# DataZooDE/anofox-forecast

Measured on AMD Instinct MI355X. Metric: series/sec fit+forecast, AutoETS h=28 on M5-shape batches, higher is better.
Workload: dtype f64

## Files before the change

### anofox-forecast_amd/csrc/ets_device.hpp

```cpp
#pragma once
#include <hip/hip_runtime.h>
#include <type_traits>
#include "det_math.hpp"
#include "nm.hpp"

namespace anofox {

enum { C_NONE = 0, C_ADD = 1, C_MUL = 2 };

constexpr double ETS_TOL = 1.0e-10;
constexpr double ETS_HUGEN = 1.0e10;
constexpr double ETS_LN2 = 0.693147180559945309417232121458;
constexpr double PAR_LO = 1.0e-4, PAR_HI = 0.9999, PHI_LO = 0.8, PHI_HI = 0.98;
constexpr int ETS_MERGED_LDS_PERIOD = 16;
constexpr int ETS_LDS_PERIOD = 64;
constexpr int ETS_MAX_PERIOD = 2048;

struct SeriesView {
    const double *y;
    size_t ld;
    int len;
    int wave_len;
    int wave_min_len;
    int rows;
    const double *yb;
    int col;
};

__device__ __forceinline__ int wave_max_i32(int v)
{
#pragma unroll
    for (int o = 32; o >= 1; o >>= 1) { int w = __shfl_xor(v, o); v = w > v ? w : v; }
    return v;
}
__device__ __forceinline__ int wave_min_i32(int v)
{
#pragma unroll
    for (int o = 32; o >= 1; o >>= 1) { int w = __shfl_xor(v, o); v = w < v ? w : v; }
    return v;
}

enum { YT_F64 = 0, YT_F32 = 1, YT_U16 = 2 };
template <class YT> struct YtCode;
template <> struct YtCode<double> { static constexpr int value = YT_F64; };
template <> struct YtCode<float> { static constexpr int value = YT_F32; };
template <> struct YtCode<unsigned short> { static constexpr int value = YT_U16; };
#ifndef ANOFOX_DM_RETRY
#define ANOFOX_DM_RETRY 0
#endif
#ifndef ANOFOX_TWO_BLOCK
#define ANOFOX_TWO_BLOCK 1
#endif
#ifndef ANOFOX_S_DM
#define ANOFOX_S_DM 8
#endif
#ifndef ANOFOX_S_GEN
#define ANOFOX_S_GEN 16
#endif
#ifndef ANOFOX_S_HBM_RING_COMPACT
#define ANOFOX_S_HBM_RING_COMPACT 16
#endif
#ifndef ANOFOX_S_COMPACT_MUL
#define ANOFOX_S_COMPACT_MUL 2
#endif
#ifndef ANOFOX_S_COMPACT_MUL_ADD
#define ANOFOX_S_COMPACT_MUL_ADD 1
#endif
#ifndef ANOFOX_K4_S_SEAS
#define ANOFOX_K4_S_SEAS 8
#endif
template <int ERR, int TREND, bool DAMPED, int SEAS>
struct EtsCfg {
    static constexpr int E = ERR, T = TREND, S = SEAS;
    static constexpr bool D = DAMPED;
    static constexpr int DIM = 1 + (TREND != C_NONE) + (SEAS != C_NONE) + (DAMPED ? 1 : 0);
    static constexpr bool ADDITIVE = (ERR == C_ADD) && (TREND != C_MUL) && (SEAS != C_MUL);
    static constexpr bool CLASSIC = false;
};

struct EtsPar { double alpha, bstar, phi, beta, gamma; DmPowLane pl; DmPowNear1 pc; };
struct EtsState { double l, b, sse, mant; int eacc; int bad; double f; double dlo, dhi, bmin; double rfar; };

template <class Cfg>
__device__ __forceinline__ void ets_unpack(const double (&x)[Cfg::DIM], EtsPar &p)
{
    int k = 0;
    p.alpha = x[k++];
    p.bstar = 0.0;
    double gstar = 0.0;
    p.phi = 1.0;
    if constexpr (Cfg::T != C_NONE) p.bstar = x[k++];
    if constexpr (Cfg::S != C_NONE) gstar = x[k++];
    if constexpr (Cfg::D) p.phi = x[k++];
    p.beta = p.alpha * p.bstar;
    p.gamma = gstar * (1.0 - p.alpha);
}

template <class Cfg, bool NEAR = false>
__device__ __forceinline__ void ets_step(const EtsPar &p, EtsState &st, double y, double &s)
{
    if constexpr (Cfg::ADDITIVE) {
        double phib = 0.0, q = st.l;
        if constexpr (Cfg::T == C_ADD) {
            phib = Cfg::D ? p.phi * st.b : st.b;
            q = st.l + phib;
        }
        double f = q;
        if constexpr (Cfg::S == C_ADD) f = q + s;
        double e = y - f;
        st.sse = fma(e, e, st.sse);
        st.l = fma(p.alpha, e, q);
        st.f = f;
        if constexpr (Cfg::T == C_ADD) st.b = fma(p.beta, e, phib);
        if constexpr (Cfg::S == C_ADD) s = fma(p.gamma, e, s);
    } else {
        double phib = 0.0, q = st.l;
        if constexpr (Cfg::T == C_ADD) {
            phib = Cfg::D ? p.phi * st.b : st.b;
            q = st.l + phib;
        } else if constexpr (Cfg::T == C_MUL) {
            if constexpr (Cfg::D) {
                const double r = st.b - 1.0;
                phib = dm_pow_near1(r, p.pc);
                if constexpr (NEAR) st.rfar = __builtin_fmax(st.rfar, fabs(r));
                else if (!(fabs(r) <= DM_POW_NEAR1_R)) {
                    if (!(st.b >= 0x1p-1000 && st.b <= 0x1p+1000)) st.bad = 1;
                    phib = dm_pow_step(st.b, p.phi, p.pl);
                }
            } else {
                st.bmin = __builtin_fmin(st.bmin, st.b);
                phib = st.b;
            }
            q = st.l * phib;
        }
        double f = q;
        if constexpr (Cfg::S == C_ADD) f = q + s;
        else if constexpr (Cfg::S == C_MUL) f = q * s;
        st.f = f;
        auto recip = [&](const double d) __attribute__((always_inline)) {
            const double ad = fabs(d);
            st.dlo = __builtin_fmin(st.dlo, ad);
            st.dhi = __builtin_fmax(st.dhi, ad);
            return dm_recip(d);
        };
        if constexpr (Cfg::E == C_MUL) {
            static_assert(Cfg::S != C_ADD, "multiplicative error with an additive season is not a valid spec");
            const double rf = recip(f);
            const double eps = (y - f) * rf;
            st.mant = st.mant * fabs(f);
            st.sse = fma(eps, eps, st.sse);
            const double qe = q * eps;
            st.l = fma(p.alpha, qe, q);
            if constexpr (Cfg::T == C_ADD) st.b = fma(p.beta, qe, phib);
            else if constexpr (Cfg::T == C_MUL) st.b = fma(p.beta, phib * eps, phib);
            if constexpr (Cfg::S == C_MUL) s = fma(p.gamma, s * eps, s);
        } else {
            const double e = y - f;
            st.sse = fma(e, e, st.sse);
            if constexpr (Cfg::S == C_MUL && Cfg::T == C_MUL) {
                const double R = recip(f * st.l);
                const double esl = e * (R * q);
                const double es = esl * st.l;
                const double sl = s * st.l;
                st.l = fma(p.alpha, es, q);
                st.b = fma(p.beta, esl, phib);
                s = fma(p.gamma, e * (R * sl), s);
            } else if constexpr (Cfg::S == C_MUL) {
                const double R = recip(f);
                const double es = e * (R * q);
                st.l = fma(p.alpha, es, q);
                if constexpr (Cfg::T == C_ADD) st.b = fma(p.beta, es, phib);
                s = fma(p.gamma, e * (R * s), s);
            } else {
                static_assert(Cfg::T == C_MUL, "general class: a multiplicative component");
                const double rl = recip(st.l);
                st.l = fma(p.alpha, e, q);
                st.b = fma(p.beta, e * rl, phib);
                if constexpr (Cfg::S == C_ADD) s = fma(p.gamma, e, s);
            }
        }
    }
}

template <class Cfg>
__device__ __forceinline__ void ets_renorm(EtsState &st)
{
    if constexpr (Cfg::E == C_MUL) {
        int ex;
        st.mant = frexp(st.mant, &ex);
        st.eacc += ex;
    }
}

template <class Cfg>
__device__ __forceinline__ double ets_objective_value(const EtsState &st, int n)
{
    if (st.bad || !(fabs(st.sse) <= 1.7976931348623157e308)) return __builtin_huge_val();
    if constexpr (!Cfg::ADDITIVE) {
        constexpr double D_LO = Cfg::E == C_MUL ? 0x1p-120 : 0x1p-1000, D_HI = Cfg::E == C_MUL ? 0x1p+120 : 0x1p+1000;
        if (n > 0 && !(st.dlo >= D_LO && st.dhi <= D_HI)) return __builtin_huge_val();
        if constexpr (Cfg::T == C_MUL && !Cfg::D) { if (n > 0 && !(st.bmin > 0.0)) return __builtin_huge_val(); }
    }
    double lik = (double)n * dm_log(st.sse);
    if constexpr (Cfg::E == C_MUL) lik = lik + 2.0 * (dm_log(st.mant) + (double)st.eacc * ETS_LN2);
    if (lik != lik) return __builtin_huge_val();
    if (lik < -1.0e10) lik = -1.0e10;
    return lik;
}

struct EtsInit {
    double l0, b0;
    const double *fig;
    size_t fig_ld;
    int m;
};

struct EtsFinalOut {
    double *yhat; int h; double *sse_out;
    double *fitted; size_t fitted_ld; double *states; size_t states_ld;
    double mean; double *var_out;
};

template <class Cfg, int MS, int K, bool FINAL, class YT = double>
__device__ __forceinline__ void ets_pass(const SeriesView &v, const EtsInit &in,
                                         const double (&cand)[K][Cfg::DIM], double (&fout)[K],
                                         double *ring, const EtsFinalOut *fin)
{
    static_assert((Cfg::S == C_NONE) == (MS == 0), "MS == 0 iff no seasonal component");
    const int lane = threadIdx.x & (NM_BLOCK - 1);
    EtsPar par[K];
    EtsState st[K];
#pragma unroll
    for (int k = 0; k < K; k++) {
        ets_unpack<Cfg>(cand[k], par[k]);
        if constexpr (Cfg::T == C_MUL && Cfg::D) { par[k].pl = dm_pow_lane(); dm_pow_near1_coef(par[k].phi, par[k].pc); }
        st[k].l = in.l0; st[k].b = in.b0; st[k].sse = 0.0; st[k].mant = 1.0; st[k].eacc = 0; st[k].bad = 0;
        st[k].f = 0.0; st[k].dlo = __builtin_huge_val(); st[k].dhi = 0.0; st[k].bmin = __builtin_huge_val(); st[k].rfar = 0.0;

    }
    const double *yp = v.yb;
    const unsigned col_bytes = (unsigned)v.col * (unsigned)sizeof(YT);
    const size_t ld = v.ld;

    const int wave_len = __builtin_amdgcn_readfirstlane(v.wave_len);
    const int wave_min_len = __builtin_amdgcn_readfirstlane(v.wave_min_len);
    const int row_max = __builtin_amdgcn_readfirstlane(v.rows) - 1;
    constexpr int S_WIDE = std::is_same_v<YT, double> ? 1 : (Cfg::ADDITIVE ? ANOFOX_S_COMPACT_MUL_ADD : ANOFOX_S_COMPACT_MUL);
    constexpr int S_FULL = (Cfg::ADDITIVE ? (K == 4 ? (MS > 0 ? ANOFOX_K4_S_SEAS : 16) : 32) : ((Cfg::T == C_MUL && Cfg::D) ? ANOFOX_S_DM : ANOFOX_S_GEN)) * S_WIDE;
    constexpr int S_HBM_CAP = (MS == -2 && !FINAL && !std::is_same_v<YT, double>) ? ANOFOX_S_HBM_RING_COMPACT : 8;
    constexpr int S_TARGET = ((MS == -2 || MS == -4) && K == 1 && S_FULL > S_HBM_CAP) ? S_HBM_CAP : S_FULL;
    constexpr int S = (MS > 0) ? ((S_TARGET / MS > 0 ? S_TARGET / MS : 1) * MS) : S_TARGET;
    typedef std::conditional_t<std::is_same_v<YT, unsigned short>, unsigned, YT> ybuf_t;
    auto widen = [](const ybuf_t x) __attribute__((always_inline)) { return (double)x; };
    ybuf_t cur[S], nxt[S];
    typedef unsigned int u32x2_t __attribute__((ext_vector_type(2)));
    const size_t row_bytes = ld * sizeof(YT);
    const size_t total_bytes = (size_t)(row_max + 1) * row_bytes;
    const int rows_total = row_max + 1;
    auto load_block = [&](ybuf_t (&buf)[S], const int row0) __attribute__((always_inline)) {
        unsigned nrec;
        size_t off;
        if constexpr (Cfg::ADDITIVE) {
            const unsigned rows_left = row0 < rows_total ? (unsigned)(rows_total - row0) : 0u;
            const unsigned long long rem = (unsigned long long)rows_left * (unsigned long long)(unsigned)row_bytes;
            nrec = (unsigned)(rem >> 32) != 0u ? 0xffffffffu : (unsigned)rem;
            off = rows_left ? (size_t)((unsigned long long)(unsigned)row0 * (unsigned long long)(unsigned)row_bytes) : (size_t)0;
        } else {
            const size_t o = (size_t)row0 * row_bytes;
            const size_t rem = o < total_bytes ? total_bytes - o : 0;
            nrec = rem > 0xffffffffull ? 0xffffffffu : (unsigned)rem;
            off = rem ? o : 0;
        }
        const auto rsrc = __builtin_amdgcn_make_buffer_rsrc((void *)((const char *)yp + off), 0, nrec, 0x00020000);
#pragma unroll
        for (int j = 0; j < S; j++) {
            if constexpr (std::is_same_v<YT, double>) {
                const u32x2_t w = __builtin_amdgcn_raw_buffer_load_b64(rsrc, col_bytes, (unsigned)(j * row_bytes), 0);
                buf[j] = __builtin_bit_cast(double, w);
            } else if constexpr (std::is_same_v<YT, float>) {
                const unsigned w = __builtin_amdgcn_raw_buffer_load_b32(rsrc, col_bytes, (unsigned)(j * row_bytes), 0);
                buf[j] = __builtin_bit_cast(float, w);
            } else {
                buf[j] = (unsigned)__builtin_amdgcn_raw_buffer_load_b16(rsrc, col_bytes, (unsigned)(j * row_bytes), 0);
            }
        }
    };
    load_block(cur, 0);
    double var_acc = 0.0;
    auto keep_fit = [&](const int t, const double yv) __attribute__((always_inline)) {
        if constexpr (FINAL) {
            if (fin->fitted && t < v.len) fin->fitted[(size_t)t * fin->fitted_ld] = st[0].f;
            const double dv = yv - fin->mean;
            var_acc += dv * dv;
        }
    };

    if constexpr (MS >= 0) {
        constexpr int MR = MS > 0 ? MS : 1;
        double s[K][MR];
        if constexpr (MS > 0) {
#pragma unroll
            for (int j = 0; j < MS; j++) {
                double f0 = in.fig[(size_t)j * in.fig_ld];
#pragma unroll
                for (int k = 0; k < K; k++) s[k][j] = f0;
            }
        } else {
#pragma unroll
            for (int k = 0; k < K; k++) s[k][0] = 0.0;
        }
        auto run_block = [&](const ybuf_t (&buf)[S], const int base, auto pred_tag) __attribute__((always_inline)) {
            constexpr bool PRED = decltype(pred_tag)::value;
            if constexpr (ANOFOX_DM_RETRY && Cfg::T == C_MUL && Cfg::D && K == 1 && !PRED && !FINAL) {
                const EtsState st0 = st[0];
                double s0[MR];
#pragma unroll
                for (int jj = 0; jj < MR; jj++) s0[jj] = s[0][jj];
                st[0].rfar = 0.0;
#pragma unroll
                for (int j = 0; j < S; j++) {
                    ets_step<Cfg, true>(par[0], st[0], widen(buf[j]), s[0][MS > 0 ? j % MR : 0]);
                    if ((j & 3) == 3 || j == S - 1) ets_renorm<Cfg>(st[0]);
                }
                const bool again = v.len > 0 && (!(st[0].rfar <= DM_POW_NEAR1_R) || st[0].b != st[0].b);
                if (__builtin_amdgcn_ballot_w64(again) == 0ull) return;
                st[0] = st0;
#pragma unroll
                for (int jj = 0; jj < MR; jj++) s[0][jj] = s0[jj];
            }
#pragma unroll
            for (int j = 0; j < S; j++) {
                if (!PRED || base + j < v.len) {
#pragma unroll
                    for (int k = 0; k < K; k++) {
                        ets_step<Cfg>(par[k], st[k], widen(buf[j]), s[k][MS > 0 ? j % MR : 0]);
                        if ((j & 3) == 3 || j == S - 1) ets_renorm<Cfg>(st[k]);
                    }
                    keep_fit(base + j, widen(buf[j]));
                }
            }
        };
        int base = 0;
        constexpr bool TWO = ANOFOX_TWO_BLOCK == 2 || (ANOFOX_TWO_BLOCK == 1 && Cfg::ADDITIVE);
        if constexpr (TWO) {
            for (; base + 2 * S <= wave_min_len; base += 2 * S) {
                load_block(nxt, base + S);
                run_block(cur, base, std::false_type{});
                load_block(cur, base + 2 * S);
                run_block(nxt, base + S, std::false_type{});
            }
        }
        for (; base < wave_len; base += S) {
            load_block(nxt, base + S);
            if (base + S <= wave_min_len) run_block(cur, base, std::false_type{});
            else run_block(cur, base, std::true_type{});
#pragma unroll
            for (int j = 0; j < S; j++) cur[j] = nxt[j];
        }
        if constexpr (FINAL) {
            if constexpr (MS > 0) {
                if (fin->states && v.len > 0) {
#pragma unroll
                    for (int jj = 0; jj < MS; jj++) fin->states[(size_t)(2 + jj) * fin->states_ld] = s[0][jj];
                }
            }
            double pp = par[0].phi, phistar = par[0].phi;
            for (int i = 0; i < fin->h; i++) {
                double f;
                if constexpr (Cfg::T == C_NONE) f = st[0].l;
                else if constexpr (Cfg::T == C_ADD) f = st[0].l + phistar * st[0].b;
                else f = (st[0].b > 0.0) ? st[0].l * dm_pow_pos(st[0].b, phistar) : __builtin_nan("");
                if constexpr (MS > 0) {
                    const int j = (v.len + i) % MS;
                    double sv = s[0][0];
#pragma unroll
                    for (int jj = 1; jj < MS; jj++) sv = (j == jj) ? s[0][jj] : sv;
                    f = (Cfg::S == C_ADD) ? f + sv : f * sv;
                }
                if (v.len > 0) fin->yhat[i] = f;
                pp = pp * par[0].phi;
                phistar = phistar + pp;
            }
        }
    } else {
        constexpr bool LANE_M = MS <= -3;
        static_assert(!LANE_M || K == 1, "per-lane periods: one candidate per lane");
        const int m = LANE_M ? in.m : __builtin_amdgcn_readfirstlane(in.m);
        const int m_max = LANE_M ? __builtin_amdgcn_readfirstlane(wave_max_i32(in.m)) : m;
        for (int j = 0; j < m_max; j++) {
            if (LANE_M && j >= m) continue;
            double f0 = in.fig[(size_t)j * in.fig_ld];
#pragma unroll
            for (int k = 0; k < K; k++) ring[(k * m + j) * NM_BLOCK + lane] = f0;
        }
        int j = 0;
        constexpr bool HBM_RING = (MS == -2 || MS == -4);
        if constexpr (HBM_RING && K == 1) {
            static_assert(2 * S <= ((MS == -2 && !FINAL) ? ETS_LDS_PERIOD : ETS_MERGED_LDS_PERIOD), "the ring prefetch needs periods of at least two blocks");
            double rc[S], rn[S];
            auto ring_load = [&](double (&buf)[S], int j0) __attribute__((always_inline)) {
#pragma unroll
                for (int i = 0; i < S; i++) {
                    buf[i] = ring[(size_t)j0 * NM_BLOCK + lane];
                    j0 = (j0 + 1 == m) ? 0 : j0 + 1;
                }
                return j0;
            };
            int jn = ring_load(rc, 0);
            int base = 0;
            for (; base < wave_len; base += S) {
                load_block(nxt, base + S);
                const int jnn = ring_load(rn, jn);
                const bool full = base + S <= wave_min_len;
#pragma unroll
                for (int i = 0; i < S; i++) {
                    if (full || base + i < v.len) {
                        double sv = rc[i];
                        ets_step<Cfg>(par[0], st[0], widen(cur[i]), sv);
                        if ((i & 3) == 3 || i == S - 1) ets_renorm<Cfg>(st[0]);
                        ring[(size_t)j * NM_BLOCK + lane] = sv;
                        keep_fit(base + i, widen(cur[i]));
                    }
                    j = (j + 1 == m) ? 0 : j + 1;
                }
#pragma unroll
                for (int i = 0; i < S; i++) { cur[i] = nxt[i]; rc[i] = rn[i]; }
                jn = jnn;
            }
        } else {
        auto ring_block = [&](const int base, const bool full) __attribute__((always_inline)) {
#pragma unroll
            for (int i = 0; i < S; i++) {
                if (full || base + i < v.len) {
#pragma unroll
                    for (int k = 0; k < K; k++) {
                        double sv = ring[(k * m + j) * NM_BLOCK + lane];
                        ets_step<Cfg>(par[k], st[k], widen(cur[i]), sv);
                        if ((i & 3) == 3 || i == S - 1) ets_renorm<Cfg>(st[k]);
                        ring[(k * m + j) * NM_BLOCK + lane] = sv;
                    }
                    keep_fit(base + i, widen(cur[i]));
                }
                j = (j + 1 == m) ? 0 : j + 1;
            }
        };
        int base = 0;
        for (; base < wave_len; base += S) {
            load_block(nxt, base + S);
            ring_block(base, base + S <= wave_min_len);
#pragma unroll
            for (int i = 0; i < S; i++) cur[i] = nxt[i];
        }
        }
        if constexpr (FINAL) {
            if (fin->states && v.len > 0)
                for (int jj = 0; jj < m; jj++) fin->states[(size_t)(2 + jj) * fin->states_ld] = ring[(0 * m + jj) * NM_BLOCK + lane];
            double pp = par[0].phi, phistar = par[0].phi;
            for (int i = 0; i < fin->h; i++) {
                double f;
                if constexpr (Cfg::T == C_NONE) f = st[0].l;
                else if constexpr (Cfg::T == C_ADD) f = st[0].l + phistar * st[0].b;
                else f = (st[0].b > 0.0) ? st[0].l * dm_pow_pos(st[0].b, phistar) : __builtin_nan("");
                const int jj = (v.len + i) % m;
                double sv = ring[(0 * m + jj) * NM_BLOCK + lane];
                f = (Cfg::S == C_ADD) ? f + sv : f * sv;
                if (v.len > 0) fin->yhat[i] = f;
                pp = pp * par[0].phi;
                phistar = phistar + pp;
            }
        }
    }
#pragma unroll
    for (int k = 0; k < K; k++) {
        ets_renorm<Cfg>(st[k]);
        fout[k] = ets_objective_value<Cfg>(st[k], v.len);
    }
    if constexpr (FINAL) {
        if (fin->sse_out && v.len > 0) *fin->sse_out = st[0].sse;
        if (fin->var_out) *fin->var_out = var_acc;
        if (fin->states && v.len > 0) { fin->states[0] = st[0].l; fin->states[fin->states_ld] = Cfg::T != C_NONE ? st[0].b : __builtin_nan(""); }
    }
}

template <class Cfg, int MS, int CPL, class YT = double>
struct EtsModel {
    static constexpr int DIM = Cfg::DIM;
    SeriesView v;
    EtsInit in;
    double *ring;
    __device__ void bounds(double (&lo)[DIM], double (&hi)[DIM], double (&x0)[DIM]) const
    {
        int k = 0;
        lo[k] = PAR_LO; hi[k] = PAR_HI; x0[k] = 0.3; k++;
        if constexpr (Cfg::T != C_NONE) { lo[k] = PAR_LO; hi[k] = PAR_HI; x0[k] = 0.1; k++; }
        if constexpr (Cfg::S != C_NONE) { lo[k] = PAR_LO; hi[k] = PAR_HI; x0[k] = 0.1; k++; }
        if constexpr (Cfg::D) { lo[k] = PHI_LO; hi[k] = PHI_HI; x0[k] = 0.9; k++; }
    }
    __device__ double eval1(const double (&x)[DIM]) const
    {
        double c1[1][DIM], f1[1];
#pragma unroll
        for (int i = 0; i < DIM; i++) c1[0][i] = x[i];
        ets_pass<Cfg, MS, 1, false, YT>(v, in, c1, f1, ring, nullptr);
        return f1[0];
    }
    __device__ void eval(const double (&cand)[NM_K][DIM], double (&f)[NM_K]) const
    {
        if constexpr (CPL == NM_K) {
            ets_pass<Cfg, MS, NM_K, false, YT>(v, in, cand, f, ring, nullptr);
        } else {
            const int sub = threadIdx.x & 3;
            double mine[1][DIM], f1[1];
#pragma unroll
            for (int i = 0; i < DIM; i++)
                mine[0][i] = sub == 0 ? cand[0][i] : (sub == 1 ? cand[1][i] : (sub == 2 ? cand[2][i] : cand[3][i]));
            ets_pass<Cfg, MS, 1, false, YT>(v, in, mine, f1, ring, nullptr);
            const int base = (threadIdx.x & (NM_BLOCK - 1)) & ~3;
#pragma unroll
            for (int k = 0; k < NM_K; k++) f[k] = __shfl(f1[0], base + k);
        }
    }
};

}
```

Baseline: 79800.

## Add optional per-row refill ring for y loads and halve renorm frequency

Adds an ANOFOX_ROW_RING option that replaces the double-buffered cur/nxt block prefetch with a single buffer, where each slot is refilled with the next block's row right after it is consumed. The goal is to cut register pressure from holding two blocks. Separately, the state renormalisation in every ETS step loop now runs every 8 steps instead of every 4, which applies unconditionally. The ring path defaults to off, so only the renorm change is active by default; it reduces work but leaves mantissa accumulation unrenormalised over longer stretches.

```diff
diff --git a/anofox-forecast_amd/csrc/ets_device.hpp b/anofox-forecast_amd/csrc/ets_device.hpp
--- a/anofox-forecast_amd/csrc/ets_device.hpp
+++ b/anofox-forecast_amd/csrc/ets_device.hpp
@@ -50,6 +50,9 @@
 #endif
 #ifndef ANOFOX_TWO_BLOCK
 #define ANOFOX_TWO_BLOCK 1
+#endif
+#ifndef ANOFOX_ROW_RING
+#define ANOFOX_ROW_RING 0
 #endif
 #ifndef ANOFOX_S_DM
 #define ANOFOX_S_DM 8
@@ -251,13 +254,16 @@
     constexpr int S_TARGET = ((MS == -2 || MS == -4) && K == 1 && S_FULL > S_HBM_CAP) ? S_HBM_CAP : S_FULL;
     constexpr int S = (MS > 0) ? ((S_TARGET / MS > 0 ? S_TARGET / MS : 1) * MS) : S_TARGET;
     typedef std::conditional_t<std::is_same_v<YT, unsigned short>, unsigned, YT> ybuf_t;
-    auto widen = [](const ybuf_t x) __attribute__((always_inline)) { return (double)x; };
-    ybuf_t cur[S], nxt[S];
+    constexpr bool ROW_RING = ANOFOX_ROW_RING && K == 1 && !ANOFOX_DM_RETRY && !(ANOFOX_ROW_RING == 2 && Cfg::T == C_MUL && Cfg::D);
+    constexpr bool RAW_RING = ROW_RING && ((MS >= 0 && Cfg::T == C_MUL && Cfg::D) || MS == -1 || MS == -3);
+    typedef std::conditional_t<RAW_RING, YT, ybuf_t> yslot_t;
+    auto widen = [](const yslot_t x) __attribute__((always_inline)) { return (double)x; };
+    yslot_t cur[S], nxt[S];
     typedef unsigned int u32x2_t __attribute__((ext_vector_type(2)));
     const size_t row_bytes = ld * sizeof(YT);
     const size_t total_bytes = (size_t)(row_max + 1) * row_bytes;
     const int rows_total = row_max + 1;
-    auto load_block = [&](ybuf_t (&buf)[S], const int row0) __attribute__((always_inline)) {
+    auto block_rsrc = [&](const int row0) __attribute__((always_inline)) {
         unsigned nrec;
         size_t off;
         if constexpr (Cfg::ADDITIVE) {
@@ -271,21 +277,43 @@
             nrec = rem > 0xffffffffull ? 0xffffffffu : (unsigned)rem;
             off = rem ? o : 0;
         }
-        const auto rsrc = __builtin_amdgcn_make_buffer_rsrc((void *)((const char *)yp + off), 0, nrec, 0x00020000);
-#pragma unroll
-        for (int j = 0; j < S; j++) {
-            if constexpr (std::is_same_v<YT, double>) {
-                const u32x2_t w = __builtin_amdgcn_raw_buffer_load_b64(rsrc, col_bytes, (unsigned)(j * row_bytes), 0);
-                buf[j] = __builtin_bit_cast(double, w);
-            } else if constexpr (std::is_same_v<YT, float>) {
-                const unsigned w = __builtin_amdgcn_raw_buffer_load_b32(rsrc, col_bytes, (unsigned)(j * row_bytes), 0);
-                buf[j] = __builtin_bit_cast(float, w);
-            } else {
-                buf[j] = (unsigned)__builtin_amdgcn_raw_buffer_load_b16(rsrc, col_bytes, (unsigned)(j * row_bytes), 0);
-            }
-        }
+        return __builtin_amdgcn_make_buffer_rsrc((void *)((const char *)yp + off), 0, nrec, 0x00020000);
+    };
+    typedef decltype(block_rsrc(0)) rsrc_t;
+    auto load_row = [&](const rsrc_t rsrc, const int j) __attribute__((always_inline)) -> yslot_t {
+        if constexpr (std::is_same_v<YT, double>) {
+            const u32x2_t w = __builtin_amdgcn_raw_buffer_load_b64(rsrc, col_bytes, (unsigned)(j * row_bytes), 0);
+            return __builtin_bit_cast(double, w);
+        } else if constexpr (std::is_same_v<YT, float>) {
+            const unsigned w = __builtin_amdgcn_raw_buffer_load_b32(rsrc, col_bytes, (unsigned)(j * row_bytes), 0);
+            return __builtin_bit_cast(float, w);
+        } else if constexpr (RAW_RING) {
+            return (unsigned short)__builtin_amdgcn_raw_buffer_load_b16(rsrc, col_bytes, (unsigned)(j * row_bytes), 0);
+        } else {
+            return (unsigned)__builtin_amdgcn_raw_buffer_load_b16(rsrc, col_bytes, (unsigned)(j * row_bytes), 0);
+        }
+    };
+    auto load_block = [&](yslot_t (&buf)[S], const int row0) __attribute__((always_inline)) {
+        const rsrc_t rsrc = block_rsrc(row0);
+#pragma unroll
+        for (int j = 0; j < S; j++) buf[j] = load_row(rsrc, j);
+    };
+    auto take_row = [&](yslot_t &slot, const rsrc_t next, const int j, auto refill_tag) __attribute__((always_inline)) {
+        double yv = widen(slot);
+        if constexpr (decltype(refill_tag)::value) {
+            asm volatile("" : "+v"(yv) : : "memory");
+            slot = load_row(next, j);
+        }
+        return yv;
     };
     load_block(cur, 0);
+    auto ring_seed = [&]() __attribute__((always_inline)) {
+        __builtin_amdgcn_s_waitcnt(0x0f70);
+        if constexpr (std::is_same_v<YT, unsigned short>) {
+#pragma unroll
+            for (int j = 0; j < S; j++) asm volatile("" : "+v"(cur[j]));
+        }
+    };
     double var_acc = 0.0;
     auto keep_fit = [&](const int t, const double yv) __attribute__((always_inline)) {
         if constexpr (FINAL) {
@@ -309,8 +337,9 @@
 #pragma unroll
             for (int k = 0; k < K; k++) s[k][0] = 0.0;
         }
-        auto run_block = [&](const ybuf_t (&buf)[S], const int base, auto pred_tag) __attribute__((always_inline)) {
-            constexpr bool PRED = decltype(pred_tag)::value;
+        auto run_block = [&](yslot_t (&buf)[S], const int base, auto pred_tag, auto refill_tag) __attribute__((always_inline)) {
+            constexpr bool PRED = decltype(pred_tag)::value, REFILL = decltype(refill_tag)::value;
+            const rsrc_t next = block_rsrc(REFILL ? base + S : 0);
             if constexpr (ANOFOX_DM_RETRY && Cfg::T == C_MUL && Cfg::D && K == 1 && !PRED && !FINAL) {
                 const EtsState st0 = st[0];
                 double s0[MR];
@@ -320,7 +349,7 @@
 #pragma unroll
                 for (int j = 0; j < S; j++) {
                     ets_step<Cfg, true>(par[0], st[0], widen(buf[j]), s[0][MS > 0 ? j % MR : 0]);
-                    if ((j & 3) == 3 || j == S - 1) ets_renorm<Cfg>(st[0]);
+                    if ((j & 7) == 7 || j == S - 1) ets_renorm<Cfg>(st[0]);
                 }
                 const bool again = v.len > 0 && (!(st[0].rfar <= DM_POW_NEAR1_R) || st[0].b != st[0].b);
                 if (__builtin_amdgcn_ballot_w64(again) == 0ull) return;
@@ -330,13 +359,14 @@
             }
 #pragma unroll
             for (int j = 0; j < S; j++) {
+                const double yv = take_row(buf[j], next, j, refill_tag);
                 if (!PRED || base + j < v.len) {
 #pragma unroll
                     for (int k = 0; k < K; k++) {
-                        ets_step<Cfg>(par[k], st[k], widen(buf[j]), s[k][MS > 0 ? j % MR : 0]);
-                        if ((j & 3) == 3 || j == S - 1) ets_renorm<Cfg>(st[k]);
+                        ets_step<Cfg>(par[k], st[k], yv, s[k][MS > 0 ? j % MR : 0]);
+                        if ((j & 7) == 7 || j == S - 1) ets_renorm<Cfg>(st[k]);
                     }
-                    keep_fit(base + j, widen(buf[j]));
+                    keep_fit(base + j, yv);
                 }
             }
         };
@@ -345,17 +375,32 @@
         if constexpr (TWO) {
             for (; base + 2 * S <= wave_min_len; base += 2 * S) {
                 load_block(nxt, base + S);
-                run_block(cur, base, std::false_type{});
+                run_block(cur, base, std::false_type{}, std::false_type{});
                 load_block(cur, base + 2 * S);
-                run_block(nxt, base + S, std::false_type{});
-            }
-        }
-        for (; base < wave_len; base += S) {
-            load_block(nxt, base + S);
-            if (base + S <= wave_min_len) run_block(cur, base, std::false_type{});
-            else run_block(cur, base, std::true_type{});
-#pragma unroll
-            for (int j = 0; j < S; j++) cur[j] = nxt[j];
+                run_block(nxt, base + S, std::false_type{}, std::false_type{});
+            }
+        }
+        if constexpr (ROW_RING && !TWO) {
+            ring_seed();
+            for (; base + S <= wave_min_len; base += S) run_block(cur, base, std::false_type{}, std::true_type{});
+            if constexpr (RAW_RING) {
+                for (; base < wave_len; base += S) run_block(cur, base, std::true_type{}, std::true_type{});
+            } else {
+                for (; base < wave_len; base += S) {
+                    load_block(nxt, base + S);
+                    run_block(cur, base, std::true_type{}, std::false_type{});
+#pragma unroll
+                    for (int j = 0; j < S; j++) cur[j] = nxt[j];
+                }
+            }
+        } else {
+            for (; base < wave_len; base += S) {
+                load_block(nxt, base + S);
+                if (base + S <= wave_min_len) run_block(cur, base, std::false_type{}, std::false_type{});
+                else run_block(cur, base, std::true_type{}, std::false_type{});
+#pragma unroll
+                for (int j = 0; j < S; j++) cur[j] = nxt[j];
+            }
         }
         if constexpr (FINAL) {
             if constexpr (MS > 0) {
@@ -417,7 +462,7 @@
                     if (full || base + i < v.len) {
                         double sv = rc[i];
                         ets_step<Cfg>(par[0], st[0], widen(cur[i]), sv);
-                        if ((i & 3) == 3 || i == S - 1) ets_renorm<Cfg>(st[0]);
+                        if ((i & 7) == 7 || i == S - 1) ets_renorm<Cfg>(st[0]);
                         ring[(size_t)j * NM_BLOCK + lane] = sv;
                         keep_fit(base + i, widen(cur[i]));
                     }
@@ -428,28 +473,33 @@
                 jn = jnn;
             }
         } else {
+        if constexpr (ROW_RING) ring_seed();
         auto ring_block = [&](const int base, const bool full) __attribute__((always_inline)) {
+            const rsrc_t next = block_rsrc(ROW_RING ? base + S : 0);
 #pragma unroll
             for (int i = 0; i < S; i++) {
+                const double yv = take_row(cur[i], next, i, std::bool_constant<ROW_RING>{});
                 if (full || base + i < v.len) {
 #pragma unroll
                     for (int k = 0; k < K; k++) {
                         double sv = ring[(k * m + j) * NM_BLOCK + lane];
-                        ets_step<Cfg>(par[k], st[k], widen(cur[i]), sv);
-                        if ((i & 3) == 3 || i == S - 1) ets_renorm<Cfg>(st[k]);
+                        ets_step<Cfg>(par[k], st[k], yv, sv);
+                        if ((i & 7) == 7 || i == S - 1) ets_renorm<Cfg>(st[k]);
                         ring[(k * m + j) * NM_BLOCK + lane] = sv;
                     }
-                    keep_fit(base + i, widen(cur[i]));
+                    keep_fit(base + i, yv);
                 }
                 j = (j + 1 == m) ? 0 : j + 1;
             }
         };
         int base = 0;
         for (; base < wave_len; base += S) {
-            load_block(nxt, base + S);
+            if constexpr (!ROW_RING) load_block(nxt, base + S);
             ring_block(base, base + S <= wave_min_len);
-#pragma unroll
-            for (int i = 0; i < S; i++) cur[i] = nxt[i];
+            if constexpr (!ROW_RING) {
+#pragma unroll
+                for (int i = 0; i < S; i++) cur[i] = nxt[i];
+            }
         }
         }
         if constexpr (FINAL) {
```

Result: no change. 79630 (median of 2 runs) (-0.2%).
